# yangdongchao/RSTnet

Hardware: AMD Instinct MI355X
Metric: codec+LM audio frames/sec (24 kHz, 12.5 Hz tokens) at batch=1 and batch=64; RVQ code-index exact-match (higher is better)
Workload: dtype f32 (large GEMMs: operands as three bf16 planes, six bf16 matrix-instruction products per fp32 product, f32 accumulate); 1 GPU; MimiCodec encode->RVQ(8x2048x256)->decode, BASELINE.json configs[1]; batch_per_gpu=64, weights=random-init (rstnet_amd.synth seed 0), parallelism=replica x1, utterances sharded, RCCL weight broadcast only

## Files before the change

rstnet_amd/csrc/b3_common.h:

```cpp
#pragma once
#include "rst_common.h"

typedef short bf16x8 __attribute__((ext_vector_type(8)));
typedef unsigned u32x2 __attribute__((ext_vector_type(2)));
typedef unsigned u32x4 __attribute__((ext_vector_type(4)));
typedef float f32x2 __attribute__((ext_vector_type(2)));
typedef __bf16 bf16x2_t __attribute__((ext_vector_type(2)));

__device__ __forceinline__ unsigned b3_peel(f32x2& v) {
    const unsigned h = __builtin_bit_cast(unsigned, __builtin_convertvector(v, bf16x2_t));
    v[0] -= __uint_as_float(h << 16);
    v[1] -= __uint_as_float(h & 0xffff0000u);
    return h;
}

template <bool MK, bool ELU>
__device__ __forceinline__ void b3_take_a(const f32x4 src, const int mask, f32x2 (&v)[2]) {
    typedef int i32x4 __attribute__((ext_vector_type(4)));
    f32x4 x = src;
    if (MK) x = __builtin_bit_cast(f32x4, __builtin_bit_cast(i32x4, x) & mask);
    if (ELU) {
        x[0] = rst_elu(x[0]); x[1] = rst_elu(x[1]); x[2] = rst_elu(x[2]); x[3] = rst_elu(x[3]);
    }
    v[0] = f32x2{x[0], x[1]};
    v[1] = f32x2{x[2], x[3]};
}

template <int TM, int TN>
__device__ __forceinline__ void b3_clear(f32x16 (&acc)[TM][TN]) {
#pragma unroll
    for (int i = 0; i < TM; ++i)
#pragma unroll
        for (int j = 0; j < TN; ++j)
#pragma unroll
            for (int e = 0; e < 16; ++e) acc[i][j][e] = 0.0f;
}

constexpr int B3_SH_ROWS = 128;

struct B3SharedTile {
    int b, t0;
    long m0, mlim;
};
struct B3SharedRow {
    unsigned ao;
    int klo, kn;
};

__host__ __device__ __forceinline__ constexpr int b3_shared_step(int R) { return B3_SH_ROWS - (R - 1); }
__host__ __device__ __forceinline__ constexpr int b3_shared_tiles_per_utt(int T_out, int R) { return (T_out + b3_shared_step(R) - 1) / b3_shared_step(R); }

__host__ __device__ __forceinline__ B3SharedTile b3_shared_tile(int mt, int R, int T_out) {
    const int tpu = b3_shared_tiles_per_utt(T_out, R), step = b3_shared_step(R);
    B3SharedTile t;
    t.b = mt / tpu;
    t.t0 = (mt - t.b * tpu) * step;
    t.m0 = (long)t.b * T_out + t.t0;
    t.mlim = (long)t.b * T_out + (t.t0 + step < T_out ? t.t0 + step : T_out);
    return t;
}

__host__ __device__ __forceinline__ B3SharedRow b3_shared_row(const B3SharedTile& t, int r, int R, int G, int TC, long x_bstride, int lk) {
    const long g = (long)t.t0 + r - (R - 1);
    const long f0 = g * G;
    B3SharedRow o;
    o.klo = 0;
    if (g < 0 || f0 >= TC) {
        o.kn = 0;
        o.ao = (unsigned)(lk * 4);
    } else {
        const long left = TC - f0;
        o.kn = (int)((left < G ? left : (long)G) / 16);
        o.ao = (unsigned)(((long)t.b * x_bstride + f0 + lk) * 4);
    }
    return o;
}

__host__ __device__ __forceinline__ unsigned b3_shared_load_offset(const B3SharedRow& row, int kt, bool& ok) {
    ok = (unsigned)kt < (unsigned)row.kn;
    return row.ao + (ok ? (unsigned)kt : 0u) * 64u;
}

#define B3_QA {2, 0, 1, 1, 0, 0}
#define B3_QB {0, 2, 1, 0, 1, 0}
```

rstnet_amd/csrc/gemm_win.hip:

```cpp
#include <algorithm>
#include "rst_common.h"
#include "rst_kernels.h"
#include "b3_common.h"

namespace {

constexpr int BK = 32;

template <int TM, int TN, bool FULL = false>
__device__ __forceinline__ void gw_epilogue(const GemmWinParams& p, const f32x16 (&acc)[TM][TN], int m0w, int n0w, int M, int lane) {
    const bool has_res = p.res != nullptr;
#pragma unroll
    for (int j = 0; j < TN; ++j) {
        const int n = n0w + j * 32 + (lane & 31);
        const bool n_ok = FULL || n < p.N;
        const float bias = (p.bias && n_ok) ? p.bias[n] : 0.0f;
        const float scale = (p.scale && n_ok) ? p.scale[n] : 1.0f;
#pragma unroll
        for (int i = 0; i < TM; ++i) {
            const int mb = m0w + i * 32 + 4 * (lane >> 5);
            const long o = (long)mb * p.ldy + n;
            float r[16];
#pragma unroll
            for (int e = 0; e < 16; ++e) {
// ... 166 lines not shown
    const int kt0 = FAST ? blockIdx.y * per_split : 0;
    const int nk = min(nk_all, kt0 + per_split);
    if (kt0 < nk) {
        load_tiles(kt0);
        store_tiles(kt0 & 1);
    }
    __syncthreads();

    const int frag_row = lane & 31;
    const int frag_k = (lane >> 5) * 4;

    auto mma_tile = [&](int buf, int ks0 = 0, int ks1 = KB / 8) {
        const float* a = As + buf * BM * LDS_LD + (wm * TM * 32 + frag_row) * LDS_LD + frag_k;
        const float* b = Bs + buf * BN * LDS_LD + (wn * TN * 32 + frag_row) * LDS_LD + frag_k;
#pragma unroll
        for (int ks = ks0; ks < ks1; ++ks) {
            f32x4 fa[TM], fb[TN];
#pragma unroll
            for (int i = 0; i < TM; ++i) fa[i] = *reinterpret_cast<const f32x4*>(a + i * 32 * LDS_LD + ks * 8);
#pragma unroll
            for (int j = 0; j < TN; ++j) fb[j] = *reinterpret_cast<const f32x4*>(b + j * 32 * LDS_LD + ks * 8);
#pragma unroll
            for (int e = 0; e < 4; ++e)
#pragma unroll
                for (int i = 0; i < TM; ++i)
#pragma unroll
                    for (int j = 0; j < TN; ++j)
                        acc[i][j] = __builtin_amdgcn_mfma_f32_32x32x2f32(fa[i][e], fb[j][e], acc[i][j], 0, 0, 0);
        }
    };

    bool interior = FAST && VEC && gridDim.y == 1 && m0 + BM <= M && n0 + BN <= p.N && p.K % KB == 0;
#pragma unroll
    for (int j = 0; j < RA; ++j) interior = interior && a_klo[j] == 0 && a_khi[j] == p.K;
    if (FAST && __syncthreads_and(interior)) {
        const float* ap[RA];
        const float* bp[RB];
#pragma unroll
        for (int j = 0; j < RA; ++j) ap[j] = p.x + a_off[j] + a_f0[j] + lk;
#pragma unroll
        for (int j = 0; j < RB; ++j) bp[j] = p.w + (long)(n0 + lrow + RP * j) * p.K + lk;
        for (int kt = kt0; kt + 1 < nk; ++kt) {
#pragma unroll
            for (int j = 0; j < RA; ++j) ra[j] = *reinterpret_cast<const f32x4*>(ap[j] + (kt + 1) * KB);
#pragma unroll
            for (int j = 0; j < RB; ++j) rb[j] = *reinterpret_cast<const f32x4*>(bp[j] + (kt + 1) * KB);
            __builtin_amdgcn_sched_barrier(0);
            mma_tile(kt & 1, 0, KB / 8 - 1);
            __builtin_amdgcn_sched_barrier(0);
            mma_tile(kt & 1, KB / 8 - 1, KB / 8);
            store_tiles((kt & 1) ^ 1, false);
#pragma unroll
            for (int g = 0; g < RA + RB; ++g) {
                __builtin_amdgcn_sched_group_barrier(0x008, (4 * TM * TN) / (RA + RB) > 0 ? (4 * TM * TN) / (RA + RB) : 1, 0);
                __builtin_amdgcn_sched_group_barrier(0x200, 1, 0);
            }
            __syncthreads();
        }
        mma_tile((nk - 1) & 1);
    } else {
        for (int kt = kt0; kt < nk; ++kt) {
            const int buf = kt & 1;
            if (kt + 1 < nk) load_tiles(kt + 1);
            __builtin_amdgcn_s_setprio(1);
            mma_tile(buf);
            __builtin_amdgcn_s_setprio(0);
            if (kt + 1 < nk) store_tiles(buf ^ 1);
            __syncthreads();
        }
    }

    if (FAST && gridDim.y > 1) {
        __shared__ int sm_last;
        float* wsb = p.ws + (long)blockIdx.y * M * p.N;
#pragma unroll
        for (int j = 0; j < TN; ++j) {
            const int n = n0 + (wn * TN + j) * 32 + (lane & 31);
#pragma unroll
            for (int i = 0; i < TM; ++i)
#pragma unroll
                for (int e = 0; e < 16; ++e) {
                    const int m = m0 + (wm * TM + i) * 32 + rst_mfma32_row(e, lane);
                    if (n < p.N && m < M)
                        __hip_atomic_store(wsb + (long)m * p.N + n, acc[i][j][e], __ATOMIC_RELAXED, __HIP_MEMORY_SCOPE_AGENT);
                }
        }
        asm volatile("s_waitcnt vmcnt(0)" ::: "memory");
        __syncthreads();
        if (tid == 0) {
            const unsigned prev = __hip_atomic_fetch_add(p.counters + tile, 1u, __ATOMIC_RELAXED, __HIP_MEMORY_SCOPE_AGENT);
            sm_last = prev == gridDim.y - 1;
            if (sm_last) __hip_atomic_store(p.counters + tile, 0u, __ATOMIC_RELAXED, __HIP_MEMORY_SCOPE_AGENT);
        }
        __syncthreads();
        if (!sm_last) return;
        constexpr int UB = TM * TN == 1 ? 8 : (TM * TN == 2 ? 4 : 1);
#pragma unroll
        for (int j = 0; j < TN; ++j) {
            const int n = min(n0 + (wn * TN + j) * 32 + (lane & 31), p.N - 1);
#pragma unroll
            for (int i = 0; i < TM; ++i) {
#pragma unroll
                for (int e = 0; e < 16; ++e) acc[i][j][e] = 0.f;
                for (int ks = 0; ks < (int)gridDim.y; ks += UB) {
                    float t[16][UB];
#pragma unroll
                    for (int e = 0; e < 16; ++e) {
                        const int m = min(m0 + (wm * TM + i) * 32 + rst_mfma32_row(e, lane), M - 1);
                        rst_load_partials<UB>(p.ws + (long)m * p.N + n, (long)M * p.N, ks, (int)gridDim.y, t[e]);
                    }
#pragma unroll
                    for (int u = 0; u < UB; ++u)
                        if (ks + u < (int)gridDim.y) {
#pragma unroll
                            for (int e = 0; e < 16; ++e) acc[i][j][e] += t[e][u];
                        }
                }
            }
        }
    }

    gw_epilogue<TM, TN>(p, acc, m0 + wm * TM * 32, n0 + wn * TN * 32, M, lane);
}

__device__ __forceinline__ int gw_xcd_first(int tiles, int x) {
    const int q = tiles >> 3, r = tiles & 7;
    return x < r ? x * (q + 1) : r * (q + 1) + (x - r) * q;
}

template <int TM, int TN, int WM, int WN, bool VEC, bool ELU, int KB>
__global__ __launch_bounds__(256) __attribute__((amdgpu_waves_per_eu(KB == 16 ? 3 : 1, KB == 16 ? 3 : 2))) void gemm_win_kernel(const GemmWinParams p) {
    extern __shared__ __attribute__((aligned(16))) float smem[];
    const int tile = gw_xcd_first(gridDim.x, blockIdx.x & 7) + (blockIdx.x >> 3);
    const int tiles_n = (p.N + 32 * TN * WN - 1) / (32 * TN * WN);
    gw_tile<TM, TN, WM, WN, VEC, ELU, KB, true>(p, tile, (tile / tiles_n) * (32 * TM * WM), (tile % tiles_n) * (32 * TN * WN), smem);
}

template <bool ELU, int KB, int DBG = 0>
__global__ __launch_bounds__(256) __attribute__((amdgpu_waves_per_eu(KB == 16 ? 3 : 1, KB == 16 ? 3 : 2))) void gemm_win_stream_kernel(const GemmWinParams p, const int tiles) {
    constexpr int TM = 2, TN = 2, WM = 2, WN = 2;
    constexpr int BM = 128, BN = 128;
    constexpr int LDS_LD = KB + 4;
    constexpr int RP = 1024 / KB;
    constexpr int RA = BM / RP, RB = BN / RP;
    extern __shared__ __attribute__((aligned(16))) float smem[];
    float* As = smem;
    float* Bs = smem + 2 * BM * LDS_LD;

    const int tid = threadIdx.x;
    const int lane = tid & 63;
    const int wave = tid >> 6;
    const int wm = wave / WN, wn = wave % WN;
    const int lrow = tid / (KB / 4);
    const int lk = (tid % (KB / 4)) * 4;
    const int frag_row = lane & 31;
    const int frag_k = (lane >> 5) * 4;

    const int M = p.B * p.T_out;
    const int TC = p.T_in * p.C;
    const int tiles_n = (p.N + BN - 1) / BN;
    const int nk = p.K / KB;
    const bool k_ok = p.K % KB == 0;

    const int xcd = blockIdx.x & 7;
    const int first = gw_xcd_first(tiles, xcd);
    const int count = gw_xcd_first(tiles, xcd + 1) - first;
    const int stride = ((int)gridDim.x + 7 - xcd) >> 3;
    int l = blockIdx.x >> 3;
    if (l >= count) return;

    struct Ctx {
        const float* ap[RA];
        unsigned bo[RB];
    };
    auto setup = [&](int m0, int n0, Ctx& c) -> bool {
        bool interior = k_ok && m0 + BM <= M && n0 + BN <= p.N;
#pragma unroll
        for (int j = 0; j < RA; ++j) {
            const int m = min(m0 + lrow + RP * j, M - 1);
            const int b = m / p.T_out;
            const int t = m - b * p.T_out;
            const int f0 = (t * p.S - p.P) * p.C;
            interior = interior && f0 >= 0 && f0 + p.K <= TC;
            c.ap[j] = p.x + (long)b * p.x_bstride + f0 + lk;
        }
#pragma unroll
        for (int j = 0; j < RB; ++j) c.bo[j] = (unsigned)min(n0 + lrow + RP * j, p.N - 1) * (unsigned)p.K + lk;
        return __syncthreads_and(interior);
    };

    f32x4 ra[RA], rb[RB];
    auto issue = [&](const Ctx& c, int kt) {
#pragma unroll
        for (int j = 0; j < RA; ++j) ra[j] = *reinterpret_cast<const f32x4*>(c.ap[j] + kt * KB);
#pragma unroll
        for (int j = 0; j < RB; ++j) rb[j] = *reinterpret_cast<const f32x4*>(p.w + c.bo[j] + kt * KB);
    };
    auto store_tiles = [&](int buf) {
        float* a = As + buf * BM * LDS_LD;
        float* b = Bs + buf * BN * LDS_LD;
#pragma unroll
        for (int j = 0; j < RA; ++j) {
            f32x4 v = ra[j];
            if (ELU) {
                v[0] = rst_elu(v[0]); v[1] = rst_elu(v[1]); v[2] = rst_elu(v[2]); v[3] = rst_elu(v[3]);
            }
            *reinterpret_cast<f32x4*>(a + (lrow + RP * j) * LDS_LD + lk) = v;
        }
#pragma unroll
        for (int j = 0; j < RB; ++j)
            *reinterpret_cast<f32x4*>(b + (lrow + RP * j) * LDS_LD + lk) = rb[j];
    };

    f32x16 acc[TM][TN];
    auto mma_tile = [&](int buf, int ks0, int ks1) {
        const float* a = As + buf * BM * LDS_LD + (wm * TM * 32 + frag_row) * LDS_LD + frag_k;
        const float* b = Bs + buf * BN * LDS_LD + (wn * TN * 32 + frag_row) * LDS_LD + frag_k;
#pragma unroll
        for (int ks = ks0; ks < ks1; ++ks) {
            f32x4 fa[TM], fb[TN];
#pragma unroll
            for (int i = 0; i < TM; ++i) fa[i] = *reinterpret_cast<const f32x4*>(a + i * 32 * LDS_LD + ks * 8);
#pragma unroll
            for (int j = 0; j < TN; ++j) fb[j] = *reinterpret_cast<const f32x4*>(b + j * 32 * LDS_LD + ks * 8);
#pragma unroll
            for (int e = 0; e < 4; ++e)
#pragma unroll
                for (int i = 0; i < TM; ++i)
#pragma unroll
                    for (int j = 0; j < TN; ++j)
                        acc[i][j] = __builtin_amdgcn_mfma_f32_32x32x2f32(fa[i][e], fb[j][e], acc[i][j], 0, 0, 0);
        }
    };
    auto step = [&](const Ctx& c, int kt, int buf) {
        if (DBG == 5) {
#pragma unroll
            for (int e = 0; e < 4 * (KB / 8); ++e)
#pragma unroll
                for (int i = 0; i < TM; ++i)
#pragma unroll
                    for (int j = 0; j < TN; ++j)
                        acc[i][j] = __builtin_amdgcn_mfma_f32_32x32x2f32(ra[0][e & 3], rb[0][e & 3], acc[i][j], 0, 0, 0);
            return;
        }
        store_tiles(buf ^ 1);
        if (DBG != 1) issue(c, kt);
        __builtin_amdgcn_sched_barrier(0);
        mma_tile(buf, 0, KB / 8);
        __syncthreads();
    };
    auto prime = [&](const Ctx& c, int buf) {
        issue(c, 0);
        store_tiles(buf);
        issue(c, 1);
        __syncthreads();
    };

    Ctx c, cn;
    int tile = first + l;
    int m0 = (tile / tiles_n) * BM, n0 = (tile % tiles_n) * BN;
    bool fast = nk >= 2 && setup(m0, n0, c);
    int buf = 0;
    if (fast) prime(c, 0);
    for (;;) {
        const bool has_next = l + stride < count;
        const int tile_n = tile + stride;
        const int m0n = (tile_n / tiles_n) * BM, n0n = (tile_n % tiles_n) * BN;
        bool fast_n = false;
        if (fast) {
            b3_clear(acc);
            int lkt = 2;
            for (int kt = 0; kt < nk; ++kt) {
                if (lkt == nk) {
                    lkt = 0;
                    if (has_next) {
                        fast_n = setup(m0n, n0n, cn);
                        if (fast_n) c = cn;
                    }
                }
                step(c, lkt, buf);
                ++lkt;
                buf ^= 1;
            }
            gw_epilogue<TM, TN, true>(p, acc, m0 + wm * TM * 32, n0 + wn * TN * 32, M, lane);
        } else {
            gw_tile<TM, TN, WM, WN, true, ELU, KB, false>(p, tile, m0, n0, smem);
            if (has_next) fast_n = nk >= 2 && setup(m0n, n0n, c);
        }
        if (!has_next) break;
        if (fast_n && !fast) prime(c, buf);
        fast = fast_n;
        l += stride;
        tile = tile_n;
        m0 = m0n;
        n0 = n0n;
    }
}


constexpr int B3_SETS_A = 4;
constexpr int B3_SETS_B = 2;
constexpr int B3_KB = 16;
constexpr int B3_RS = 24;

template <int V>
struct b3_int { static constexpr int value = V; };

__host__ __device__ __forceinline__ constexpr int b3_row(int g) { return (g & ~7) | (2 * (g & 3) + ((g >> 2) & 1)); }

template <bool ELU, bool MASK, int NWN, int DBG = 0>
__global__ __launch_bounds__(128 * NWN) __attribute__((amdgpu_waves_per_eu(2, 2))) void gemm_win_b3_stream_kernel(const GemmWinParams p, const int tiles) {
    constexpr int TM = 2, TN = 2;
    constexpr int NT = 128 * NWN;
    constexpr int BM = 128, BN = 64 * NWN;
    constexpr int RA = 512 / NT;
    constexpr int A_PLANE = BM * B3_RS;
    constexpr int BUF = 3 * A_PLANE;
    constexpr int NSA = B3_SETS_A, NSB = B3_SETS_B;
    static_assert(NSA == 4 && NSB == 2, "the rotation below is written out for four activation sets and two weight sets");
    static_assert(NWN == 2 || NWN == 4, "two or four waves along N");
    extern __shared__ __attribute__((aligned(16))) float smem[];
    short* const lds = reinterpret_cast<short*>(smem);

    const int tid = threadIdx.x;
    const int lane = tid & 63;
    const int wave = tid >> 6;
    const int wm = wave / NWN, wn = wave % NWN;
    const int lrow = b3_row(tid >> 2);
    const int lk = (tid & 3) * 4;
    const int frag_row = lane & 31;
    const int frag_k = (lane >> 5) * 8;

    const int M = p.B * p.T_out;
    const int TC = p.T_in * p.C;
    const int tiles_n = (p.N + BN - 1) / BN;
    const int nk = p.K / B3_KB;

    const int xcd = blockIdx.x & 7;
    const int first = gw_xcd_first(tiles, xcd);
    const int count = gw_xcd_first(tiles, xcd + 1) - first;
    const int stride = ((int)gridDim.x + 7 - xcd) >> 3;
    int l = blockIdx.x >> 3;
    if (l >= count) return;

    struct Ctx {
        unsigned ao[RA];
        int klo[RA], kn[RA];
    };
    auto setup = [&](int m0, Ctx& c) {
#pragma unroll
        for (int j = 0; j < RA; ++j) {
            const int m = m0 + lrow + (NT / 4) * j;
            const int mm = min(m, M - 1);
            const int b = mm / p.T_out;
            const int t = mm - b * p.T_out;
            const int f0 = (t * p.S - p.P) * p.C;
            long off = (long)b * p.x_bstride + f0 + lk;
            if (MASK) {
                int klo = max(0, -f0) / B3_KB, khi = min(p.K, TC - f0) / B3_KB;
                if (m >= M || klo >= khi) {
                    klo = khi = 0;
                    off = lk;
                }
                c.klo[j] = klo;
                c.kn[j] = khi - klo;
                off += (long)klo * B3_KB;
            }
            c.ao[j] = (unsigned)(off * 4);
        }
    };
    auto w_tile = [&](int n0) { return (unsigned)(n0 / 32) * (unsigned)nk * 3072u; };
    const unsigned wo = (unsigned)(wn * TN) * (unsigned)nk * 3072u + (unsigned)lane * 16u;
    const unsigned wo_blk = (unsigned)nk * 3072u;

    f32x4 ra[NSA][RA];
    int rm[NSA][RA];
    u32x4 rw[NSB][TN][3];
    const int a_dst = lrow * B3_RS + lk;
    const int a_frag = (wm * TM * 32 + frag_row) * B3_RS + frag_k;

    const __amdgpu_buffer_rsrc_t rs_x = __builtin_amdgcn_make_buffer_rsrc(const_cast<float*>(p.x), 0, 0xffffffff, 0x00020000);
    const __amdgpu_buffer_rsrc_t rs_w = __builtin_amdgcn_make_buffer_rsrc(const_cast<short*>(p.w3), 0, 0xffffffff, 0x00020000);
    auto load_a = [&](auto MM, const Ctx& c, const int kt, f32x4 (&dst)[RA], int (&mask)[RA]) {
        constexpr bool MK = decltype(MM)::value != 0;
#pragma unroll
        for (int j = 0; j < RA; ++j) {
            if (MK) {
                const unsigned d = (unsigned)(kt - c.klo[j]);
                const bool ok = d < (unsigned)c.kn[j];
                mask[j] = ok ? -1 : 0;
                const unsigned vo = c.ao[j] + (ok ? d : 0u) * (B3_KB * 4);
                dst[j] = __builtin_bit_cast(f32x4, __builtin_amdgcn_raw_buffer_load_b128(rs_x, vo, 0, 0));
            } else {
                dst[j] = __builtin_bit_cast(f32x4, __builtin_amdgcn_raw_buffer_load_b128(rs_x, c.ao[j], kt * (B3_KB * 4), 0));
            }
        }
    };
    auto load_wq = [&](auto UU, auto QQ, const unsigned wb, const int kt) {
        constexpr int U = decltype(UU)::value, q = decltype(QQ)::value;
#pragma unroll
        for (int j = 0; j < TN; ++j) {
            const unsigned so = wb + (unsigned)kt * 3072u + q * 1024u;
            rw[U][j][q] = __builtin_amdgcn_raw_buffer_load_b128(rs_w, wo + j * wo_blk, so, 0);
        }
    };

    f32x16 acc[TM][TN];

    auto stage = [&](auto SS, auto MM, const Ctx& c, const int kta, const unsigned bp, const int ktb, const int buf) {
        constexpr int S = decltype(SS)::value;
        constexpr int F = (S + 3) % 4, SB = S % 2;
        if (DBG != 2 && DBG != 3) load_a(MM, c, kta, ra[F], rm[F]);
        bf16x8 fa[TM][3];
        const short* rd = lds + buf * BUF;
        short* wr = lds + (buf ^ 1) * BUF;
        constexpr int QA[6] = {2, 1, 0, 0, 1, 0};
        constexpr int QB[6] = {0, 0, 0, 2, 1, 1};
        if (DBG != 3) {
#pragma unroll
            for (int i = 0; i < TM; ++i) fa[i][2] = *reinterpret_cast<const bf16x8*>(rd + a_frag + 2 * A_PLANE + i * 32 * B3_RS);
#pragma unroll
            for (int i = 0; i < TM; ++i) fa[i][1] = *reinterpret_cast<const bf16x8*>(rd + a_frag + A_PLANE + i * 32 * B3_RS);
#pragma unroll
            for (int i = 0; i < TM; ++i) fa[i][0] = *reinterpret_cast<const bf16x8*>(rd + a_frag + i * 32 * B3_RS);
        } else {
#pragma unroll
            for (int q = 0; q < 3; ++q)
#pragma unroll
                for (int i = 0; i < TM; ++i) fa[i][q] = __builtin_bit_cast(bf16x8, ra[S][0]);
        }
        __builtin_amdgcn_sched_barrier(0);

        f32x2 v[RA][2];
        u32x2 h[RA];
        constexpr bool SIDE = DBG != 1 && DBG != 3;
        constexpr int PB = 2 * RA + 1, NOPS = 3 * PB;
#pragma unroll
        for (int m = 0; m < 24; ++m) {
            const int t = m >> 2, i = (m >> 1) & 1, j = m & 1;
            acc[i][j] = __builtin_amdgcn_mfma_f32_32x32x16_bf16(fa[i][QA[t]], __builtin_bit_cast(bf16x8, rw[SB][j][QB[t]]), acc[i][j], 0, 0, 0);
            if (DBG != 2 && DBG != 3) {
                if (m == 11) load_wq(b3_int<SB>{}, b3_int<0>{}, bp, ktb);
                if (m == 15) load_wq(b3_int<SB>{}, b3_int<2>{}, bp, ktb);
                if (m == 23) load_wq(b3_int<SB>{}, b3_int<1>{}, bp, ktb);
            }
            if (SIDE && m == 0) {
#pragma unroll
                for (int r = 0; r < RA; ++r) b3_take_a<decltype(MM)::value != 0, ELU>(ra[S][r], rm[S][r], v[r]);
            }
            const int op = RA == 2 ? m - 1 : ((m & 1) ? (m - 1) >> 1 : -1);
            if (SIDE && op >= 0 && op < NOPS) {
                const int q = op / PB, w = op % PB;
                if (w < 2 * RA) {
                    if (DBG == 5) h[w >> 1][w & 1] = __builtin_bit_cast(unsigned, v[w >> 1][w & 1][0]) + q;
                    else h[w >> 1][w & 1] = b3_peel(v[w >> 1][w & 1]);
                } else {
#pragma unroll
                    for (int r = 0; r < RA; ++r) *reinterpret_cast<u32x2*>(wr + a_dst + q * A_PLANE + r * (NT / 4) * B3_RS) = h[r];
                }
            }
            __builtin_amdgcn_sched_barrier(0);
        }
        if (DBG != 4) __syncthreads();
    };

    auto prime = [&](const Ctx& c, const unsigned bp, int buf) {
        short* wr = lds + buf * BUF;
        {
            f32x4 xa[RA];
            int xm[RA];
            load_a(b3_int<MASK>{}, c, 0, xa, xm);
#pragma unroll
            for (int j = 0; j < RA; ++j) {
                f32x2 v[2];
                b3_take_a<MASK, ELU>(xa[j], xm[j], v);
#pragma unroll
                for (int q = 0; q < 3; ++q) {
                    u32x2 hh;
                    hh[0] = b3_peel(v[0]);
                    hh[1] = b3_peel(v[1]);
                    *reinterpret_cast<u32x2*>(wr + a_dst + q * A_PLANE + j * (NT / 4) * B3_RS) = hh;
                }
            }
        }
        load_wq(b3_int<0>{}, b3_int<0>{}, bp, 0); load_wq(b3_int<0>{}, b3_int<2>{}, bp, 0); load_wq(b3_int<0>{}, b3_int<1>{}, bp, 0);
        load_wq(b3_int<1>{}, b3_int<0>{}, bp, 1); load_wq(b3_int<1>{}, b3_int<2>{}, bp, 1); load_wq(b3_int<1>{}, b3_int<1>{}, bp, 1);
#pragma unroll
        for (int g = 1; g < 4; ++g) load_a(b3_int<MASK>{}, c, g, ra[g - 1], rm[g - 1]);
        __syncthreads();
    };

    Ctx c;
    int tile = first + l;
    int m0 = (tile / tiles_n) * BM, n0 = (tile % tiles_n) * BN;
    setup(m0, c);
    unsigned bp = w_tile(n0);
    unsigned bpn = bp;
    int kb = 2;
    prime(c, bp, 0);
    for (;;) {
        const int ln = l + stride;
        const bool has_next = ln < count;
        const int tile_n = first + ln;
        const int m0n = (tile_n / tiles_n) * BM, n0n = (tile_n % tiles_n) * BN;
        b3_clear(acc);
        int kf = 4;
        auto cross = [&]() {
            kf = 0;
            if (has_next) {
                setup(m0n, c);
                bpn = w_tile(n0n);
            }
        };
        constexpr b3_int<MASK> MM{};
        for (int kt = 0; kt < nk; kt += 4) {
            if (kf == nk) cross();
            stage(b3_int<0>{}, MM, c, kf, bp, kb, 0);
            stage(b3_int<1>{}, MM, c, kf + 1, bp, kb + 1, 1);
            kb += 2;
            if (kb == nk) {
                kb = 0;
                bp = bpn;
            }
            stage(b3_int<2>{}, MM, c, kf + 2, bp, kb, 0);
            stage(b3_int<3>{}, MM, c, kf + 3, bp, kb + 1, 1);
            kb += 2;
            if (kb == nk) {
                kb = 0;
                bp = bpn;
            }
            kf += 4;
        }
        if (!MASK || (m0 + BM <= M && n0 + BN <= p.N)) gw_epilogue<TM, TN, true>(p, acc, m0 + wm * TM * 32, n0 + wn * TN * 32, M, lane);
        else gw_epilogue<TM, TN, false>(p, acc, m0 + wm * TM * 32, n0 + wn * TN * 32, M, lane);
        if (!has_next) break;
        l = ln;
        tile = tile_n;
        m0 = m0n;
        n0 = n0n;
    }
}

template <int TM, int TN>
__device__ __forceinline__ void gw_epilogue_rows(const GemmWinParams& p, const f32x16 (&acc)[TM][TN], long m0, int rows, int rw, int n0w, int lane) {
    const bool has_res = p.res != nullptr;
    const unsigned bytes = (unsigned)rows * (unsigned)p.ldy * 4u;
    const __amdgpu_buffer_rsrc_t rs_y = __builtin_amdgcn_make_buffer_rsrc(p.y + m0 * p.ldy, 0, bytes, 0x00020000);
    const __amdgpu_buffer_rsrc_t rs_r = __builtin_amdgcn_make_buffer_rsrc(const_cast<float*>(has_res ? p.res + m0 * p.ldy : p.y), 0, has_res ? bytes : 0u, 0x00020000);
    const unsigned row_bytes = (unsigned)p.ldy * 4u;
#pragma unroll
    for (int j = 0; j < TN; ++j) {
        const int n = n0w + j * 32 + (lane & 31);
        const float bias = p.bias ? p.bias[n] : 0.0f;
        const float scale = p.scale ? p.scale[n] : 1.0f;
#pragma unroll
        for (int i = 0; i < TM; ++i) {
            const unsigned o = (unsigned)(rw + i * 32 + 4 * (lane >> 5)) * row_bytes + (unsigned)n * 4u;
            float r[16];
#pragma unroll
            for (int e = 0; e < 16; ++e) {
                const unsigned dm = (e & 3) + 8 * (e >> 2);
                r[e] = has_res ? __uint_as_float(__builtin_amdgcn_raw_buffer_load_b32(rs_r, o + dm * row_bytes, 0, 0)) : 0.0f;
            }
#pragma unroll
            for (int e = 0; e < 16; ++e) {
                const unsigned dm = (e & 3) + 8 * (e >> 2);
                float v = acc[i][j][e] + bias;
                if (p.act_out == 1) v = rst_gelu(v);
                if (has_res) v = r[e] + scale * v;
                if (p.act_out == 2) v = rst_elu(v);
                __builtin_amdgcn_raw_buffer_store_b32(__float_as_uint(v), rs_y, o + dm * row_bytes, 0, 0);
            }
        }
    }
}

template <bool ELU, int NWN, int R>
__global__ __launch_bounds__(128 * NWN) __attribute__((amdgpu_waves_per_eu(2, 2))) void gemm_win_b3_stream_shared_kernel(const GemmWinParams p, const int tiles) {
    constexpr int TM = 2, TN = 2;
    constexpr int NT = 128 * NWN;
    constexpr int BN = 64 * NWN;
    constexpr int RA = 512 / NT;
    constexpr int A_PLANE = (B3_SH_ROWS + R - 1) * B3_RS;
    constexpr int BUF = 3 * A_PLANE;
    constexpr int NSA = B3_SETS_A;
    static_assert(NSA == 4 && B3_SETS_B == 2, "the rotation below is written out for four activation sets and two weight sets");
    static_assert(R == 2 || R == 3, "two or three taps");
    extern __shared__ __attribute__((aligned(16))) float smem[];
    short* const lds = reinterpret_cast<short*>(smem);

    const int tid = threadIdx.x;
    const int lane = tid & 63;
    const int wave = tid >> 6;
    const int wm = wave / NWN, wn = wave % NWN;
    const int lrow = b3_row(tid >> 2);
    const int lk = (tid & 3) * 4;
    const int frag_row = lane & 31;
    const int frag_k = (lane >> 5) * 8;

    const int G = p.S * p.C;
    const int TC = p.T_in * p.C;
    const int tiles_n = (p.N + BN - 1) / BN;
    const int nkg = G / B3_KB;
    const int nk = R * nkg;

    const int xcd = blockIdx.x & 7;
    const int first = gw_xcd_first(tiles, xcd);
    const int count = gw_xcd_first(tiles, xcd + 1) - first;
    const int stride = ((int)gridDim.x + 7 - xcd) >> 3;
    int l = blockIdx.x >> 3;
    if (l >= count) return;

    struct Ctx {
        B3SharedRow row[RA];
    };
    auto setup = [&](const int tile, Ctx& c) {
        const B3SharedTile ti = b3_shared_tile(tile / tiles_n, R, p.T_out);
#pragma unroll
        for (int j = 0; j < RA; ++j) c.row[j] = b3_shared_row(ti, lrow + (NT / 4) * j, R, G, TC, p.x_bstride, lk);
    };
    auto w_tile = [&](int n0) { return (unsigned)(n0 / 32) * (unsigned)nk * 3072u; };
    const unsigned wo = (unsigned)(wn * TN) * (unsigned)nk * 3072u + (unsigned)lane * 16u;
    const unsigned wo_blk = (unsigned)nk * 3072u;

    f32x4 ra[NSA][RA];
    int rm[NSA][RA];
    u32x4 rw[2][TN][3];
    const int a_dst = lrow * B3_RS + lk;
    const int a_frag = (wm * TM * 32 + frag_row) * B3_RS + frag_k;

    const __amdgpu_buffer_rsrc_t rs_x = __builtin_amdgcn_make_buffer_rsrc(const_cast<float*>(p.x), 0, 0xffffffff, 0x00020000);
    const __amdgpu_buffer_rsrc_t rs_w = __builtin_amdgcn_make_buffer_rsrc(const_cast<short*>(p.w3), 0, 0xffffffff, 0x00020000);
    auto load_a = [&](const Ctx& c, const int kt, f32x4 (&dst)[RA], int (&mask)[RA]) {
#pragma unroll
        for (int j = 0; j < RA; ++j) {
            bool ok;
            const unsigned vo = b3_shared_load_offset(c.row[j], kt, ok);
            mask[j] = ok ? -1 : 0;
            dst[j] = __builtin_bit_cast(f32x4, __builtin_amdgcn_raw_buffer_load_b128(rs_x, vo, 0, 0));
        }
    };
    auto load_wq = [&](const int u, const int q, const unsigned wb, const int pk) {
#pragma unroll
        for (int j = 0; j < TN; ++j) {
            const unsigned so = wb + (unsigned)pk * 3072u + q * 1024u;
            rw[u][j][q] = __builtin_amdgcn_raw_buffer_load_b128(rs_w, wo + j * wo_blk, so, 0);
        }
    };

    f32x16 acc[TM][TN];

    auto stage = [&](auto SS, const Ctx& c, const int kta, const unsigned bp, const unsigned bpn, const int kt, const int buf) {
        constexpr int S = decltype(SS)::value;
        constexpr int F = (S + 3) % 4;
        load_a(c, kta, ra[F], rm[F]);
        bf16x8 fa[TM][3];
        const short* rd = lds + buf * BUF + a_frag;
        short* wr = lds + (buf ^ 1) * BUF + a_dst;
        constexpr int QA[6] = {2, 1, 0, 0, 1, 0};
        constexpr int QB[6] = {0, 0, 0, 2, 1, 1};
#pragma unroll
        for (int q = 2; q >= 0; --q)
#pragma unroll
            for (int i = 0; i < TM; ++i) fa[i][q] = *reinterpret_cast<const bf16x8*>(rd + q * A_PLANE + i * 32 * B3_RS);
        __builtin_amdgcn_sched_barrier(0);

        f32x2 v[RA][2];
        u32x2 hh[RA];
        constexpr int PB = 2 * RA + 1, NOPS = 3 * PB, SP = R * (RA == 2 ? 1 : 2);
#pragma unroll
        for (int mm = 0; mm < 24 * R; ++mm) {
            const int h = mm / 24, m = mm % 24;
            const int t = m >> 2, i = (m >> 1) & 1, j = m & 1;
            const int u = (R * S + h) & 1;
            acc[i][j] = __builtin_amdgcn_mfma_f32_32x32x16_bf16(fa[i][QA[t]], __builtin_bit_cast(bf16x8, rw[u][j][QB[t]]), acc[i][j], 0, 0, 0);
            if (m == 11 || m == 15 || m == 23) {
                const int h2 = (h + 2) % R, dk = (h + 2) / R;
                const bool over = dk != 0 && kt + dk == nkg;
                load_wq(u, m == 11 ? 0 : (m == 15 ? 2 : 1), over ? bpn : bp, (over ? 0 : kt + dk) + h2 * nkg);
            }
            if (h + 1 < R && (m == 3 || m == 19 || m == 23)) {
                const int q = m == 3 ? 2 : (m == 19 ? 1 : 0);
#pragma unroll
                for (int ii = 0; ii < TM; ++ii) fa[ii][q] = *reinterpret_cast<const bf16x8*>(rd + (h + 1) * B3_RS + q * A_PLANE + ii * 32 * B3_RS);
            }
            if (mm == 0) {
#pragma unroll
                for (int r = 0; r < RA; ++r) b3_take_a<true, ELU>(ra[S][r], rm[S][r], v[r]);
            }
            const int op = (mm >= 1 && (mm - 1) % SP == 0) ? (mm - 1) / SP : -1;
            if (op >= 0 && op < NOPS) {
                const int q = op / PB, w = op % PB;
                if (w < 2 * RA) {
                    hh[w >> 1][w & 1] = b3_peel(v[w >> 1][w & 1]);
                } else {
#pragma unroll
                    for (int r = 0; r < RA; ++r) *reinterpret_cast<u32x2*>(wr + q * A_PLANE + r * (NT / 4) * B3_RS) = hh[r];
                }
            }
            __builtin_amdgcn_sched_barrier(0);
        }
        __syncthreads();
    };

    if (tid < 2 * 3 * (R - 1) * 3) {
        const int piece = tid % 3, row = tid / 3;
        const int b = row / (3 * (R - 1)), q = (row / (R - 1)) % 3, e = row % (R - 1);
        *reinterpret_cast<u32x4*>(lds + b * BUF + q * A_PLANE + (B3_SH_ROWS + e) * B3_RS + piece * 8) = u32x4{0u, 0u, 0u, 0u};
    }

    Ctx c;
    int tile = first + l;
    int n0 = (tile % tiles_n) * BN;
    setup(tile, c);
    unsigned bp = w_tile(n0);
    unsigned bpn = bp;
    {
        f32x4 xa[RA];
        int xm[RA];
        load_a(c, 0, xa, xm);
#pragma unroll
        for (int j = 0; j < RA; ++j) {
            f32x2 v[2];
            b3_take_a<true, ELU>(xa[j], xm[j], v);
#pragma unroll
            for (int q = 0; q < 3; ++q) {
                u32x2 hh;
                hh[0] = b3_peel(v[0]);
                hh[1] = b3_peel(v[1]);
                *reinterpret_cast<u32x2*>(lds + a_dst + q * A_PLANE + j * (NT / 4) * B3_RS) = hh;
            }
        }
        load_wq(0, 0, bp, 0); load_wq(0, 2, bp, 0); load_wq(0, 1, bp, 0);
        load_wq(1, 0, bp, nkg); load_wq(1, 2, bp, nkg); load_wq(1, 1, bp, nkg);
#pragma unroll
        for (int g = 1; g < 4; ++g) load_a(c, g, ra[g - 1], rm[g - 1]);
        __syncthreads();
    }
    for (;;) {
        const int ln = l + stride;
        const bool has_next = ln < count;
        const int tile_n = first + ln;
        const B3SharedTile ti = b3_shared_tile(tile / tiles_n, R, p.T_out);
        b3_clear(acc);
        int kf = 4;
        for (int kt = 0; kt < nkg; kt += 4) {
            if (kf == nkg) {
                kf = 0;
                if (has_next) {
                    setup(tile_n, c);
                    bpn = w_tile((tile_n % tiles_n) * BN);
                }
            }
            stage(b3_int<0>{}, c, kf, bp, bpn, kt, 0);
            stage(b3_int<1>{}, c, kf + 1, bp, bpn, kt + 1, 1);
            stage(b3_int<2>{}, c, kf + 2, bp, bpn, kt + 2, 0);
            stage(b3_int<3>{}, c, kf + 3, bp, bpn, kt + 3, 1);
            kf += 4;
        }
        bp = bpn;
        if (n0 + BN <= p.N) gw_epilogue_rows<TM, TN>(p, acc, ti.m0, (int)(ti.mlim - ti.m0), wm * TM * 32, n0 + wn * TN * 32, lane);
        else gw_epilogue<TM, TN, false>(p, acc, (int)ti.m0 + wm * TM * 32, n0 + wn * TN * 32, (int)ti.mlim, lane);
        if (!has_next) break;
        l = ln;
        tile = tile_n;
        n0 = (tile % tiles_n) * BN;
    }
}

__global__ __launch_bounds__(256) void gemm_win_b3_pack_kernel(const float* __restrict__ w, short* __restrict__ w3, int N, int K, long total) {
    const long i = (long)blockIdx.x * 256 + threadIdx.x;
    if (i >= total) return;
    const int kq = K / 4;
    const int n = (int)(i / kq);
    const int k = (int)(i % kq) * 4;
    f32x4 v = {0.f, 0.f, 0.f, 0.f};
    if (n < N) v = *reinterpret_cast<const f32x4*>(w + (long)n * K + k);
    f32x2 v0 = {v[0], v[1]}, v1 = {v[2], v[3]};
    short* dst = w3 + ((long)(n / 32) * (K / B3_KB) + k / B3_KB) * (3 * 512) + ((n % 32) + 32 * ((k % B3_KB) / 8)) * 8 + k % 8;
#pragma unroll
    for (int q = 0; q < 3; ++q) {
        u32x2 h;
        h[0] = b3_peel(v0);
        h[1] = b3_peel(v1);
        *reinterpret_cast<u32x2*>(dst + q * 512) = h;
    }
}


template <int TM, int TN, int WM, int WN, int KB = BK>
int launch_cfg(const GemmWinParams& p, bool vec, hipStream_t stream) {
    constexpr int BM = 32 * TM * WM, BN = 32 * TN * WN;
    const long M = (long)p.B * p.T_out;
    const long tiles = ((M + BM - 1) / BM) * ((p.N + BN - 1) / BN);
    if (tiles <= 0) return RST_OK;
    if (tiles > 0x7fffffffL) {
        rst_set_error("gemm_win: too many tiles (%ld)", tiles);
        return RST_ERR_UNSUPPORTED;
    }
    const size_t lds = 2 * (BM + BN) * (KB + 4) * sizeof(float);
    auto go = [&](auto k) {
        constexpr auto kern = decltype(k)::fn;
        rst_allow_dynamic_lds<kern>(128 * 1024);
        hipLaunchKernelGGL(kern, dim3((unsigned)tiles, (unsigned)(p.split_k > 1 ? p.split_k : 1)), dim3(256), lds, stream, p);
    };
    const bool elu = p.act_in == 1;
    if (vec && elu) go(RstKernel<gemm_win_kernel<TM, TN, WM, WN, true, true, KB>>{});
    else if (vec) go(RstKernel<gemm_win_kernel<TM, TN, WM, WN, true, false, KB>>{});
    else if (elu) go(RstKernel<gemm_win_kernel<TM, TN, WM, WN, false, true, KB>>{});
    else go(RstKernel<gemm_win_kernel<TM, TN, WM, WN, false, false, KB>>{});
    return rst_check_launch("gemm_win");
}

static int gw_cu_count() {
    return rst_cu_count();
}

template <int KB>
int launch_stream(const GemmWinParams& p, long tiles, hipStream_t stream) {
    if (tiles > 0x7fffffffL) {
        rst_set_error("gemm_win: too many tiles (%ld)", tiles);
        return RST_ERR_UNSUPPORTED;
    }
    const size_t lds = 2 * (128 + 128) * (KB + 4) * sizeof(float);
    static const int per_cu_env = rst_knob("RST_GEMM_STREAM_WGS", 0);
    const int per_cu = per_cu_env > 0 ? per_cu_env : (KB == 16 ? 3 : 2);
    const long resident = (long)per_cu * gw_cu_count();
    const unsigned grid = (unsigned)(tiles < resident ? tiles : resident);
    auto go = [&](auto k) {
        constexpr auto kern = decltype(k)::fn;
        rst_allow_dynamic_lds<kern>(128 * 1024);
        hipLaunchKernelGGL(kern, dim3(grid), dim3(256), lds, stream, p, (int)tiles);
    };
#ifdef RST_ABLATION
    static const int dbg = rst_knob("RST_GEMM_DBG", 0);
    if (KB == 16 && dbg == 1) { go(RstKernel<gemm_win_stream_kernel<false, 16, 1>>{}); return rst_check_launch("gemm_win"); }
    if (KB == 16 && dbg == 5) { go(RstKernel<gemm_win_stream_kernel<false, 16, 5>>{}); return rst_check_launch("gemm_win"); }
#endif
    if (p.act_in == 1) go(RstKernel<gemm_win_stream_kernel<true, KB>>{});
    else go(RstKernel<gemm_win_stream_kernel<false, KB>>{});
    return rst_check_launch("gemm_win");
}

static int b3_shared_taps(const GemmWinParams& p) {
    const long G = (long)p.S * p.C;
    if (G % 64 != 0 || p.K % G != 0) return 0;
    const long R = p.K / G;
    if ((R != 2 && R != 3) || p.P != (R - 1) * p.S) return 0;
    return (int)R;
}

template <int NWN, int R>
int launch_shared_b3_cfg(const GemmWinParams& p, hipStream_t stream) {
    constexpr int BN = 64 * NWN;
    const long tiles = (long)p.B * b3_shared_tiles_per_utt(p.T_out, R) * ((p.N + BN - 1) / BN);
    if (tiles > 0x7fffffffL) {
        rst_set_error("gemm_win: too many tiles (%ld)", tiles);
        return RST_ERR_UNSUPPORTED;
    }
    const size_t lds = 2 * 3 * (B3_SH_ROWS + R - 1) * B3_RS * sizeof(short);
    const long resident = (long)(NWN == 2 ? 2 : 1) * gw_cu_count();
    const unsigned grid = (unsigned)(tiles < resident ? tiles : resident);
    if (p.act_in == 1) hipLaunchKernelGGL((gemm_win_b3_stream_shared_kernel<true, NWN, R>), dim3(grid), dim3(128 * NWN), lds, stream, p, (int)tiles);
    else hipLaunchKernelGGL((gemm_win_b3_stream_shared_kernel<false, NWN, R>), dim3(grid), dim3(128 * NWN), lds, stream, p, (int)tiles);
    return rst_check_launch("gemm_win_b3");
}

template <int NWN>
int launch_stream_b3_cfg(const GemmWinParams& p, hipStream_t stream) {
    constexpr int BN = 64 * NWN;
    const long M = (long)p.B * p.T_out;
    const long tiles = ((M + 127) / 128) * ((p.N + BN - 1) / BN);
    if (tiles > 0x7fffffffL) {
        rst_set_error("gemm_win: too many tiles (%ld)", tiles);
        return RST_ERR_UNSUPPORTED;
    }
    const size_t lds = 2 * 3 * 128 * B3_RS * sizeof(short);
    static const int per_cu = rst_knob("RST_B3_WGS", NWN == 2 ? 2 : 1);
    const long resident = (long)per_cu * gw_cu_count();
    const unsigned grid = (unsigned)(tiles < resident ? tiles : resident);
    auto go = [&](auto k) {
        constexpr auto kern = decltype(k)::fn;
        rst_allow_dynamic_lds<kern>(128 * 1024);
        hipLaunchKernelGGL(kern, dim3(grid), dim3(128 * NWN), lds, stream, p, (int)tiles);
    };
    bool lean = p.P == 0 && M % 128 == 0 && p.N % BN == 0 && (long)(p.T_out - 1) * p.S * p.C + p.K <= (long)p.T_in * p.C;
#ifdef RST_ABLATION
    static const int force_mask = rst_knob("RST_B3_FORCE_MASK", 0);
    if (force_mask) lean = false;
    static const int dbg = rst_knob("RST_B3_DBG", 0);
    if (dbg == 1) { go(RstKernel<gemm_win_b3_stream_kernel<false, true, NWN, 1>>{}); return rst_check_launch("gemm_win_b3"); }
    if (dbg == 2) { go(RstKernel<gemm_win_b3_stream_kernel<false, true, NWN, 2>>{}); return rst_check_launch("gemm_win_b3"); }
    if (dbg == 3) { go(RstKernel<gemm_win_b3_stream_kernel<false, true, NWN, 3>>{}); return rst_check_launch("gemm_win_b3"); }
    if (dbg == 4) { go(RstKernel<gemm_win_b3_stream_kernel<false, true, NWN, 4>>{}); return rst_check_launch("gemm_win_b3"); }
    if (dbg == 5) { go(RstKernel<gemm_win_b3_stream_kernel<false, true, NWN, 5>>{}); return rst_check_launch("gemm_win_b3"); }
#endif
    static const int share = rst_knob("RST_B3_SHARE", 1);
    if (share) {
        const int taps = b3_shared_taps(p);
        if (taps == 2) return launch_shared_b3_cfg<NWN, 2>(p, stream);
        if (taps == 3) return launch_shared_b3_cfg<NWN, 3>(p, stream);
    }
    if (p.act_in == 1) {
        if (lean) go(RstKernel<gemm_win_b3_stream_kernel<true, false, NWN>>{});
        else go(RstKernel<gemm_win_b3_stream_kernel<true, true, NWN>>{});
    } else {
        if (lean) go(RstKernel<gemm_win_b3_stream_kernel<false, false, NWN>>{});
        else go(RstKernel<gemm_win_b3_stream_kernel<false, true, NWN>>{});
    }
    return rst_check_launch("gemm_win_b3");
}

int launch_stream_b3(const GemmWinParams& p, hipStream_t stream) {
    static const int wide_knob = rst_knob("RST_B3_WIDE", 1);
    const int waste = ((p.N + 255) / 256) * 256 - p.N;
    const long wide_tiles = (((long)p.B * p.T_out + 127) / 128) * ((p.N + 255) / 256);
    if (wide_knob && p.N >= 256 && waste * 8 <= p.N && wide_tiles >= 2L * gw_cu_count()) return launch_stream_b3_cfg<4>(p, stream);
    return launch_stream_b3_cfg<2>(p, stream);
}

}

static int gw_tile_cfg(long M, int N) {
    if (N > 64) return M > 4096 ? 0 : 1;
    if (N > 32) return 2;
    return 3;
}
static void gw_tile_dims(int cfg, int& BM, int& BN) {
    BM = cfg == 0 ? 128 : cfg == 1 ? 32 : cfg == 2 ? 128 : 256;
    BN = cfg == 0 ? 128 : cfg == 1 ? 128 : cfg == 2 ? 64 : 32;
}

int rst_gemm_split_plan_impl(long M, int N, int K) {
    if (M <= 0 || M > 4096 || (M <= 32 && N <= 64)) return 1;
    int BM, BN;
    gw_tile_dims(gw_tile_cfg(M, N), BM, BN);
    const long tiles = ((M + BM - 1) / BM) * ((N + BN - 1) / BN);
    const int nk = (K + BK - 1) / BK;
    int s = 1;
    while (tiles * s * 2 <= 256 && nk / (2 * s) >= 2 && s < 64) s *= 2;
    return s;
}

bool rst_gemm_win_b3_shape_ok(int B, int T_in, int T_out, int C, int K, int N, int pad_mode, long x_bstride, bool has_hist) {
    if (B <= 0 || T_in <= 0 || T_out <= 0 || C <= 0 || K <= 0 || N <= 0) return false;
    const long M = (long)B * T_out;
    if (gw_tile_cfg(M, N) != 0) return false;
    if (K % 64 != 0 || C % 16 != 0 || x_bstride % 4 != 0 || has_hist || pad_mode != 0) return false;
    const long x_bytes = ((long)(B - 1) * x_bstride + (long)T_in * C) * 4;
    const long w_bytes = rst_gemm_win_b3_weight_elems_impl(N, K) * 2;
    return x_bytes < 0xfffff000L && w_bytes < 0xfffff000L;
}

int rst_launch_gemm_win(const GemmWinParams& p, hipStream_t stream) {
    RST_REQUIRE(p.B >= 0 && p.T_in >= 0 && p.T_out >= 0 && p.C > 0 && p.K > 0 && p.N > 0 && p.S > 0 && p.P >= 0,
                "gemm_win: bad sizes B=%d T_in=%d T_out=%d C=%d K=%d N=%d S=%d P=%d", p.B, p.T_in, p.T_out, p.C,
                p.K, p.N, p.S, p.P);
    if (p.B == 0 || p.T_out == 0) return RST_OK;
    RST_REQUIRE(p.w && p.y && (p.x || p.T_in == 0), "gemm_win: null pointer");
    RST_REQUIRE((long)p.T_in * p.C < 0x7fffffffL && (long)p.T_out * p.S * p.C < 0x7fffffffL,
                "gemm_win: per-batch activation too large for 32-bit indexing");
    const bool vec = (p.C % 4 == 0) && (p.K % 4 == 0) && (p.x_bstride % 4 == 0) &&
                     ((uintptr_t)p.x % 16 == 0) && ((uintptr_t)p.w % 16 == 0) &&
                     (!p.hist || (uintptr_t)p.hist % 16 == 0);
    const long M = (long)p.B * p.T_out;
    RST_REQUIRE(p.split_k <= 1 || (p.ws && p.counters && M <= 4096), "gemm_win: split-K needs M <= 4096 and the scratch buffers");
    RST_REQUIRE(!p.w3 || gw_tile_cfg(M, p.N) == 0, "gemm_win_b3: %ld x %d is not a large-launch shape (more than 4096 rows, N > 64)", M, p.N);
    switch (gw_tile_cfg(M, p.N)) {
        case 0: {
            const long tiles = ((M + 127) / 128) * ((p.N + 127) / 128);
            static const bool kb32_only = rst_knob("RST_GEMM_KB32", 0) != 0;
            static const bool stream_off = rst_knob("RST_GEMM_STREAM", 1) == 0;
            if (p.w3) {
                RST_REQUIRE(vec && p.split_k <= 1 && (uintptr_t)p.w3 % 16 == 0 &&
                            rst_gemm_win_b3_shape_ok(p.B, p.T_in, p.T_out, p.C, p.K, p.N, p.pad_mode, p.x_bstride, p.hist != nullptr),
                            "gemm_win_b3: shape / alignment not served by the three-plane kernel (B=%d T_in=%d T_out=%d C=%d K=%d N=%d pad=%d "
                            "hist=%d); ask rst_gemm_win_b3_supported", p.B, p.T_in, p.T_out, p.C, p.K, p.N, p.pad_mode, p.hist != nullptr);
                return launch_stream_b3(p, stream);
            }
            static const int under_knob = rst_knob("RST_GEMM_UNDERFILL", 1);
            if (under_knob && tiles < gw_cu_count() && p.split_k <= 1) return launch_cfg<1, 1, 1, 4>(p, vec, stream);
            if (vec && !stream_off && p.split_k <= 1) {
                if (tiles >= 768 && !kb32_only) return launch_stream<16>(p, tiles, stream);
                return launch_stream<32>(p, tiles, stream);
            }
            if (tiles >= 768 && !kb32_only) return launch_cfg<2, 2, 2, 2, 16>(p, vec, stream);
            return launch_cfg<2, 2, 2, 2>(p, vec, stream);
        }
        case 1: return launch_cfg<1, 1, 1, 4>(p, vec, stream);
        case 2: return launch_cfg<1, 2, 4, 1>(p, vec, stream);
        default: return launch_cfg<2, 1, 4, 1>(p, vec, stream);
    }
}

int rst_gemm_split_tiles_impl(long M, int N) {
    int BM, BN;
    gw_tile_dims(gw_tile_cfg(M, N), BM, BN);
    return (int)(((M + BM - 1) / BM) * ((N + BN - 1) / BN));
}

long rst_gemm_win_b3_weight_elems_impl(int N, int K) { return (long)((N + 255) / 256) * 256 * K * 3; }

int rst_launch_gemm_win_b3_pack(const float* w, unsigned short* w3, int N, int K, hipStream_t stream) {
    RST_REQUIRE(w && w3 && N > 0 && K > 0 && K % 16 == 0, "gemm_win_b3_pack_weight: bad arguments (K %% 16 == 0 required, N=%d K=%d)", N, K);
    RST_REQUIRE((uintptr_t)w % 16 == 0 && (uintptr_t)w3 % 16 == 0, "gemm_win_b3_pack_weight: pointers must be 16-byte aligned");
    const long total = (long)((N + 255) / 256) * 256 * (K / 4);
    hipLaunchKernelGGL(gemm_win_b3_pack_kernel, dim3((unsigned)((total + 255) / 256)), dim3(256), 0, stream, w, reinterpret_cast<short*>(w3), N, K, total);
    return rst_check_launch("gemm_win_b3_pack_weight");
}
```

Measured before the change: 196,500 frames/s.

## Stagger half the waves by a half-stage in the eight-wave b3 stream GEMM

Adds a staggered schedule for the eight-wave (NWN=4) b3 streamed GEMM. One role of waves runs offset by half a K stage, so its MFMA bursts overlap the other role's LDS writes, bf16 peeling and barrier waits. Wave-to-tile mapping is remapped, and constexpr checks verify that no rotated wave reads an LDS buffer while it is being written. It is on by default for lean (unmasked) shapes. An optional s_setprio variant is reachable only through ablation knobs. The cost is a large hand-scheduled code path, higher register pressure, and risk of subtle ordering bugs.

```diff
diff --git a/rstnet_amd/csrc/b3_common.h b/rstnet_amd/csrc/b3_common.h
--- a/rstnet_amd/csrc/b3_common.h
+++ b/rstnet_amd/csrc/b3_common.h
@@ -83,3 +83,35 @@
 
 #define B3_QA {2, 0, 1, 1, 0, 0}
 #define B3_QB {0, 2, 1, 0, 1, 0}
+
+__host__ __device__ __forceinline__ constexpr int b3_stg_role(int mode, int wave) { return mode == 1 ? (wave >> 2) & 1 : (mode == 2 ? wave & 1 : 0); }
+__host__ __device__ __forceinline__ constexpr int b3_stg_wm(int mode, int wave, int nwn) { return mode == 1 ? (wave >> 1) & 1 : (mode == 2 ? (wave >> 2) & 1 : wave / nwn); }
+__host__ __device__ __forceinline__ constexpr int b3_stg_wn(int mode, int wave, int nwn) {
+    return mode == 1 ? (wave & 1) + 2 * (wave >> 2) : (mode == 2 ? ((wave >> 1) & 1) + 2 * (wave & 1) : wave % nwn);
+}
+__host__ __device__ __forceinline__ constexpr int b3_stg_intervals(int role, int n) { return n + role; }
+__host__ __device__ __forceinline__ constexpr bool b3_stg_has_barrier(int i, int n) { return i < n; }
+__host__ __device__ __forceinline__ constexpr int b3_stg_half(int role, int i, int slot, int n) {
+    const int stage = role ? i - 1 + slot : i;
+    const int half = role ? 1 - slot : slot;
+    return stage < 0 || stage >= n ? -1 : 2 * stage + half;
+}
+__host__ __device__ __forceinline__ constexpr int b3_stg_half_products(int R) { return 12 * R; }
+__host__ __device__ __forceinline__ constexpr int b3_stg_buf(int stage, int nbuf) { return stage % nbuf; }
+__host__ __device__ __forceinline__ constexpr int b3_stg_write_buf(int i, int nbuf) { return (i + 1) % nbuf; }
+__host__ __device__ __forceinline__ constexpr bool b3_stg_slot_reads_lds(int role, int slot, int nbuf) { return !(role == 1 && slot == 0 && nbuf == 2); }
+__host__ __device__ __forceinline__ constexpr unsigned b3_stg_read_set(int role, int i, int n, int nbuf) {
+    unsigned set = 0;
+    for (int slot = 0; slot < 2; ++slot) {
+        const int hs = b3_stg_half(role, i, slot, n);
+        if (hs >= 0 && b3_stg_slot_reads_lds(role, slot, nbuf)) set |= 1u << b3_stg_buf(hs >> 1, nbuf);
+    }
+    return set;
+}
+__host__ __device__ __forceinline__ constexpr bool b3_stg_tile_ends(int half_stage, int nk) { return half_stage >= 0 && (half_stage + 1) % (2 * nk) == 0; }
+__host__ __device__ __forceinline__ constexpr bool b3_stg_lds_legal(int n, int nbuf) {
+    for (int i = 0; i < n; ++i)
+        for (int role = 0; role < 2; ++role)
+            if (b3_stg_read_set(role, i, n, nbuf) >> b3_stg_write_buf(i, nbuf) & 1u) return false;
+    return true;
+}
diff --git a/rstnet_amd/csrc/gemm_win.hip b/rstnet_amd/csrc/gemm_win.hip
--- a/rstnet_amd/csrc/gemm_win.hip
+++ b/rstnet_amd/csrc/gemm_win.hip
@@ -492,15 +492,19 @@
 constexpr int B3_SETS_B = 2;
 constexpr int B3_KB = 16;
 constexpr int B3_RS = 24;
+constexpr int B3_STAGGER_LEAN = 1;
+constexpr int B3_STAGGER_MASKED = 0;
 
 template <int V>
 struct b3_int { static constexpr int value = V; };
 
 __host__ __device__ __forceinline__ constexpr int b3_row(int g) { return (g & ~7) | (2 * (g & 3) + ((g >> 2) & 1)); }
 
-template <bool ELU, bool MASK, int NWN, int DBG = 0>
+template <bool ELU, bool MASK, int NWN, int DBG = 0, int STG = 0, int PRIO = 0>
 __global__ __launch_bounds__(128 * NWN) __attribute__((amdgpu_waves_per_eu(2, 2))) void gemm_win_b3_stream_kernel(const GemmWinParams p, const int tiles) {
     constexpr int TM = 2, TN = 2;
+    static_assert((STG == 0 && PRIO == 0) || (NWN == 4 && DBG == 0), "stagger / priority: the eight-wave form, no ablation");
+    static_assert(STG == 0 || (b3_stg_lds_legal(4, 2) && b3_stg_lds_legal(7, 2)), "a rotated wave would read a buffer that is being written");
     constexpr int NT = 128 * NWN;
     constexpr int BM = 128, BN = 64 * NWN;
     constexpr int RA = 512 / NT;
@@ -515,7 +519,7 @@
     const int tid = threadIdx.x;
     const int lane = tid & 63;
     const int wave = tid >> 6;
-    const int wm = wave / NWN, wn = wave % NWN;
+    const int wm = STG == 0 ? wave / NWN : b3_stg_wm(STG, wave, NWN), wn = STG == 0 ? wave % NWN : b3_stg_wn(STG, wave, NWN);
     const int lrow = b3_row(tid >> 2);
     const int lk = (tid & 3) * 4;
     const int frag_row = lane & 31;
@@ -688,6 +692,136 @@
     unsigned bpn = bp;
     int kb = 2;
     prime(c, bp, 0);
+    if constexpr (PRIO != 0) {
+        if (__builtin_amdgcn_readfirstlane(wave >> 2)) __builtin_amdgcn_s_setprio(1);
+    }
+    if constexpr (STG != 0) {
+        if (__builtin_amdgcn_readfirstlane(b3_stg_role(STG, wave))) {
+            constexpr b3_int<MASK> MM{};
+            constexpr int QA[6] = {2, 1, 0, 0, 1, 0};
+            constexpr int QB[6] = {0, 0, 0, 2, 1, 1};
+            constexpr int PB = 2 * RA + 1, NOPS = 3 * PB;
+            bf16x8 fr[TM][3];
+            f32x2 v[RA][2];
+            u32x2 h[RA];
+            auto side = [&](auto SS, const int op) __attribute__((always_inline)) {
+                constexpr int S = decltype(SS)::value;
+                short* wr = lds + b3_stg_write_buf(S, 2) * BUF;
+                if (op == -1) {
+#pragma unroll
+                    for (int r = 0; r < RA; ++r) b3_take_a<MASK, ELU>(ra[S][r], rm[S][r], v[r]);
+                }
+                if (op >= 0 && op < NOPS) {
+                    const int q = op / PB, w = op % PB;
+                    if (w < 2 * RA) {
+                        h[w >> 1][w & 1] = b3_peel(v[w >> 1][w & 1]);
+                    } else {
+#pragma unroll
+                        for (int r = 0; r < RA; ++r) *reinterpret_cast<u32x2*>(wr + a_dst + q * A_PLANE + r * (NT / 4) * B3_RS) = h[r];
+                    }
+                }
+            };
+            auto frag = [&](auto SS, const int q) __attribute__((always_inline)) {
+                const short* rd = lds + b3_stg_buf(decltype(SS)::value, 2) * BUF + a_frag;
+#pragma unroll
+                for (int i = 0; i < TM; ++i) fr[i][q] = *reinterpret_cast<const bf16x8*>(rd + q * A_PLANE + i * 32 * B3_RS);
+            };
+            auto half = [&](auto SS, auto WS, const int m0h, const int slot0, const bool spread, const bool refill, const unsigned bpw, const int ktw)
+                            __attribute__((always_inline)) {
+                constexpr int S = decltype(SS)::value, SB = S % 2;
+#pragma unroll
+                for (int e = 0; e < b3_stg_half_products(1); ++e) {
+                    const int m = m0h + e;
+                    const int t = m >> 2, i = (m >> 1) & 1, j = m & 1;
+                    acc[i][j] = __builtin_amdgcn_mfma_f32_32x32x16_bf16(fr[i][QA[t]], __builtin_bit_cast(bf16x8, rw[SB][j][QB[t]]), acc[i][j], 0, 0, 0);
+                    if (m == 11) load_wq(b3_int<SB>{}, b3_int<0>{}, bpw, ktw);
+                    if (m == 15 && slot0 >= 0) load_wq(b3_int<SB>{}, b3_int<2>{}, bpw, ktw);
+                    if (m == 23 && slot0 >= 0) load_wq(b3_int<SB>{}, b3_int<1>{}, bpw, ktw);
+                    if (refill && m == 19) frag(b3_int<(S + 1) % 4>{}, 1);
+                    if (refill && m == 23) frag(b3_int<(S + 1) % 4>{}, 0);
+                    if (slot0 >= 0) {
+                        const int s = slot0 + e;
+                        if (spread) side(WS, s == 0 ? -1 : (RA == 2 ? s - 1 : ((s & 1) ? (s - 1) >> 1 : -2)));
+                        else side(WS, e - 1);
+                    }
+                    __builtin_amdgcn_sched_barrier(0);
+                }
+            };
+            auto interval = [&](auto SS, const Ctx& cc, const int kta, const unsigned bpb, const int ktbb, const unsigned bpa, const int ktba)
+                                __attribute__((always_inline)) {
+                constexpr int S = decltype(SS)::value;
+                static_assert(b3_stg_half(1, S + 4, 0, 8) == 2 * (S + 3) + 1 && b3_stg_half(1, S + 4, 1, 8) == 2 * (S + 4), "slot order of the rotated role");
+                load_a(MM, cc, kta, ra[(S + 3) % 4], rm[(S + 3) % 4]);
+                frag(SS, 2);
+                __builtin_amdgcn_sched_barrier(0);
+                half(b3_int<(S + 3) % 4>{}, SS, 12, 0, true, true, bpb, ktbb);
+                half(SS, SS, 0, 12, true, false, bpa, ktba);
+                __syncthreads();
+            };
+            auto head = [&](const Ctx& cc, const int kta, const unsigned bpa, const int ktba) __attribute__((always_inline)) {
+                load_a(MM, cc, kta, ra[3], rm[3]);
+                frag(b3_int<0>{}, 2);
+                frag(b3_int<0>{}, 1);
+                frag(b3_int<0>{}, 0);
+                __builtin_amdgcn_sched_barrier(0);
+                half(b3_int<0>{}, b3_int<0>{}, 0, 0, false, false, bpa, ktba);
+                __syncthreads();
+            };
+            unsigned bpo = bp;
+            int kbo = kb;
+            auto weights_on = [&]() {
+                bpo = bp;
+                kbo = kb;
+                kb += 2;
+                if (kb == nk) {
+                    kb = 0;
+                    bp = bpn;
+                }
+            };
+            for (;;) {
+                const int ln = l + stride;
+                const bool has_next = ln < count;
+                const int tile_n = first + ln;
+                const int m0n = (tile_n / tiles_n) * BM, n0n = (tile_n % tiles_n) * BN;
+                b3_clear(acc);
+                int kf = 4;
+                auto cross = [&]() {
+                    kf = 0;
+                    if (has_next) {
+                        setup(m0n, c);
+                        bpn = w_tile(n0n);
+                    }
+                };
+                if (kf == nk) cross();
+                head(c, kf, bp, kb);
+                interval(b3_int<1>{}, c, kf + 1, bp, kb, bp, kb + 1);
+                weights_on();
+                interval(b3_int<2>{}, c, kf + 2, bpo, kbo + 1, bp, kb);
+                interval(b3_int<3>{}, c, kf + 3, bp, kb, bp, kb + 1);
+                weights_on();
+                kf += 4;
+                for (int kt = 4; kt < nk; kt += 4) {
+                    if (kf == nk) cross();
+                    interval(b3_int<0>{}, c, kf, bpo, kbo + 1, bp, kb);
+                    interval(b3_int<1>{}, c, kf + 1, bp, kb, bp, kb + 1);
+                    weights_on();
+                    interval(b3_int<2>{}, c, kf + 2, bpo, kbo + 1, bp, kb);
+                    interval(b3_int<3>{}, c, kf + 3, bp, kb, bp, kb + 1);
+                    weights_on();
+                    kf += 4;
+                }
+                half(b3_int<3>{}, b3_int<0>{}, 12, -1, false, false, bpo, kbo + 1);
+                if (!MASK || (m0 + BM <= M && n0 + BN <= p.N)) gw_epilogue<TM, TN, true>(p, acc, m0 + wm * TM * 32, n0 + wn * TN * 32, M, lane);
+                else gw_epilogue<TM, TN, false>(p, acc, m0 + wm * TM * 32, n0 + wn * TN * 32, M, lane);
+                if (!has_next) return;
+                load_wq(b3_int<1>{}, b3_int<2>{}, bpo, kbo + 1);
+                load_wq(b3_int<1>{}, b3_int<1>{}, bpo, kbo + 1);
+                l = ln;
+                m0 = m0n;
+                n0 = n0n;
+            }
+        }
+    }
     for (;;) {
         const int ln = l + stride;
         const bool has_next = ln < count;
@@ -1091,12 +1225,35 @@
         if (taps == 2) return launch_shared_b3_cfg<NWN, 2>(p, stream);
         if (taps == 3) return launch_shared_b3_cfg<NWN, 3>(p, stream);
     }
-    if (p.act_in == 1) {
-        if (lean) go(RstKernel<gemm_win_b3_stream_kernel<true, false, NWN>>{});
-        else go(RstKernel<gemm_win_b3_stream_kernel<true, true, NWN>>{});
+    auto run = [&](auto stg_lean, auto stg_masked, auto prio) {
+        constexpr int GL = decltype(stg_lean)::value, GM = decltype(stg_masked)::value, PR = decltype(prio)::value;
+        if (p.act_in == 1) {
+            if (lean) go(RstKernel<gemm_win_b3_stream_kernel<true, false, NWN, 0, GL, PR>>{});
+            else go(RstKernel<gemm_win_b3_stream_kernel<true, true, NWN, 0, GM, PR>>{});
+        } else {
+            if (lean) go(RstKernel<gemm_win_b3_stream_kernel<false, false, NWN, 0, GL, PR>>{});
+            else go(RstKernel<gemm_win_b3_stream_kernel<false, true, NWN, 0, GM, PR>>{});
+        }
+    };
+    if constexpr (NWN == 4) {
+#ifdef RST_ABLATION
+        static const int stg_knob = rst_knob("RST_B3_STAGGER", -1), prio_knob = rst_knob("RST_B3_PRIO", 0);
+        if (prio_knob) {
+            if (stg_knob == 1) run(b3_int<1>{}, b3_int<1>{}, b3_int<1>{});
+            else if (stg_knob == 2) run(b3_int<2>{}, b3_int<2>{}, b3_int<1>{});
+            else run(b3_int<0>{}, b3_int<0>{}, b3_int<1>{});
+            return rst_check_launch("gemm_win_b3");
+        }
+        if (stg_knob >= 0) {
+            if (stg_knob == 1) run(b3_int<1>{}, b3_int<1>{}, b3_int<0>{});
+            else if (stg_knob == 2) run(b3_int<2>{}, b3_int<2>{}, b3_int<0>{});
+            else run(b3_int<0>{}, b3_int<0>{}, b3_int<0>{});
+            return rst_check_launch("gemm_win_b3");
+        }
+#endif
+        run(b3_int<B3_STAGGER_LEAN>{}, b3_int<B3_STAGGER_MASKED>{}, b3_int<0>{});
     } else {
-        if (lean) go(RstKernel<gemm_win_b3_stream_kernel<false, false, NWN>>{});
-        else go(RstKernel<gemm_win_b3_stream_kernel<false, true, NWN>>{});
+        run(b3_int<0>{}, b3_int<0>{}, b3_int<0>{});
     }
     return rst_check_launch("gemm_win_b3");
 }
```

Result: no change. 195,900 frames/s (-0.3%).
